# lmcinnes/pynndescent

Measured on AMD Instinct MI355X. Metric: index build: points indexed/sec (recall@10 vs brute force reported alongside), higher is better.
Workload: dtype f32

## Files before the change

include/pynnd_amd.h:

```cpp
#ifndef PYNND_AMD_H
#define PYNND_AMD_H

#include <stdint.h>

#ifdef __cplusplus
extern "C" {
#endif

#define NND_METRIC_SQEUCLIDEAN 0
#define NND_METRIC_ALT_COSINE 1
#define NND_METRIC_ALT_DOT 2
#define NND_METRIC_ALT_INNER_PRODUCT 3
#define NND_METRIC_CORRELATION 4
#define NND_METRIC_ALT_HELLINGER 5
enum { NND_METRIC_PROXY_INNER_PRODUCT = 6 };
enum {
    NND_METRIC_JACCARD = 8,
    NND_METRIC_DICE = 9,
    NND_METRIC_SOKALSNEATH = 10,
    NND_METRIC_MATCHING = 11,
    NND_METRIC_ROGERSTANIMOTO = 12,
    NND_METRIC_SOKALMICHENER = 13,
    NND_METRIC_KULSINSKI = 14,
    NND_METRIC_RUSSELLRAO = 15,
// ... 12 lines not shown
    int32_t n_trees;
    int32_t leaf_size;
    int32_t max_depth;
    int32_t max_candidates;
    int32_t n_iters;
    float delta;
    int64_t rng_state[3];
    int64_t tree_rng[3];
    int32_t device;
    int32_t join_blocks;
    int32_t flags;
    int32_t reserved[5];
} nnd_params;

#define NND_FLAG_NO_GRAPH 1
#define NND_FLAG_NO_PREP 2
#define NND_FLAG_TEST_SELECT_WAVE 4
#define NND_FLAG_TEST_SMALL_REGIONS 8
#define NND_FLAG_TEST_ROUTE_PLAIN 16
#define NND_FLAG_TEST_FOREST_BY_TREE 32
#define NND_FLAG_TEST_FAIL 64
#define NND_FLAG_TEST_VANISH 128
#define NND_FLAG_TEST_SAMPLE_ATOMIC 256
#define NND_FLAG_TEST_FOREST_FALLBACK_TOPS 512
#define NND_FLAG_TEST_FOREST_FALLBACK_SHARE 1024
#define NND_TEST_FALLBACK_AT(flags) ((((flags) & 512) ? 1 : 0) + (((flags) & 1024) ? 2 : 0))
#define NND_FLAG_TEST_SAMPLE_NOMEM 2048
#define NND_FLAG_TEST_SELECT_HALF 4096
#define NND_FLAG_TEST_GATHER_INLINE 8192
#define NND_FLAG_TEST_JOIN_UNSTAGED 16384

#define NND_FLAG_TEST_EXACT_F64 32768
#define NND_FLAG_TEST_RANDOM_INIT_ROWWISE 65536

typedef struct nnd_stats {
    int64_t n_iters_run;
    int64_t n_leaves;
    int64_t tree_levels;
    int64_t leaf_pairs;
    int64_t leaf_rows;
    int64_t join_pairs[64];
    int64_t join_rows[64];
    int64_t join_active[64];
    int64_t proposals[64];
    int64_t updates[64];
    float ms_prep, ms_forest, ms_leaf_init, ms_random_init, ms_descent, ms_finalize;
    float ms_sample[64], ms_join[64], ms_merge[64];
    int64_t join_mfma[64];
    int64_t leaf_mfma;
    int64_t n_cells;
    int64_t join_substeps[64];
} nnd_stats;

int32_t nnd_abi_version(void);
const char *nnd_last_global_error(void);
const char *nnd_last_error(nnd_handle_t h);

int32_t nnd_create(nnd_handle_t *out, const nnd_params *params);
int32_t nnd_destroy(nnd_handle_t h);
int32_t nnd_release_pending(void);

int32_t nnd_host_copy(void *dst, const void *src, int64_t bytes);
int32_t nnd_host_sqrt_f32(float *dst, const float *src, int64_t count);
void *nnd_host_alloc(int64_t bytes);
int32_t nnd_host_free(void *p);

// ... 254 lines not shown
```

pynndescent_amd/_capi.py:

```python
import ctypes as C
import os

import numpy as np

_HERE = os.path.dirname(os.path.abspath(__file__))
LIB_PATH = os.environ.get("PYNND_AMD_LIB", os.path.join(_HERE, "libpynnd_amd.so"))

NND_METRIC_SQEUCLIDEAN = 0
NND_METRIC_ALT_COSINE = 1
NND_METRIC_ALT_DOT = 2
NND_METRIC_ALT_INNER_PRODUCT = 3
NND_METRIC_CORRELATION = 4
NND_METRIC_ALT_HELLINGER = 5
NND_METRIC_PROXY_INNER_PRODUCT = 6
METRIC_CODES = {"euclidean": NND_METRIC_SQEUCLIDEAN, "l2": NND_METRIC_SQEUCLIDEAN, "sqeuclidean": NND_METRIC_SQEUCLIDEAN,
                "cosine": NND_METRIC_ALT_COSINE, "dot": NND_METRIC_ALT_DOT, "inner_product": NND_METRIC_ALT_INNER_PRODUCT,
                "correlation": NND_METRIC_CORRELATION, "hellinger": NND_METRIC_ALT_HELLINGER,
                "proxy_inner_product": NND_METRIC_PROXY_INNER_PRODUCT}
(NND_METRIC_JACCARD, NND_METRIC_DICE, NND_METRIC_SOKALSNEATH, NND_METRIC_MATCHING, NND_METRIC_ROGERSTANIMOTO,
 NND_METRIC_SOKALMICHENER, NND_METRIC_KULSINSKI, NND_METRIC_RUSSELLRAO, NND_METRIC_YULE) = range(8, 17)
BOOLEAN_METRIC_CODES = {"jaccard": NND_METRIC_JACCARD, "dice": NND_METRIC_DICE, "sokalsneath": NND_METRIC_SOKALSNEATH,
                        "matching": NND_METRIC_MATCHING, "rogerstanimoto": NND_METRIC_ROGERSTANIMOTO,
                        "sokalmichener": NND_METRIC_SOKALMICHENER, "kulsinski": NND_METRIC_KULSINSKI,
                        "russellrao": NND_METRIC_RUSSELLRAO, "yule": NND_METRIC_YULE}


def metric_code(name):
    return METRIC_CODES[name] if name in METRIC_CODES else BOOLEAN_METRIC_CODES[name]
NND_DTYPE_FLOAT32, NND_DTYPE_FLOAT16, NND_DTYPE_BFLOAT16, NND_DTYPE_FLOAT64 = 0, 1, 2, 3
NND_FILTER_MASK, NND_FILTER_IDS = 0, 1
NND_QUERY_FORMS = {"float": 0, "proxy": 1, "rerank": 2}
NND_CORRECT_COPY, NND_CORRECT_SQRT, NND_CORRECT_ALT_COSINE, NND_CORRECT_ALT_INNER_PRODUCT, NND_CORRECT_ALT_HELLINGER = 0, 1, 2, 3, 4
NND_LINEAR_DIAGONAL, NND_LINEAR_DENSE = 0, 1
NND_FLAG_NO_GRAPH = 1
NND_FLAG_NO_PREP = 2
NND_FLAG_TEST_SELECT_WAVE = 4
NND_FLAG_TEST_SMALL_REGIONS = 8
NND_FLAG_TEST_ROUTE_PLAIN = 16
NND_FLAG_TEST_FOREST_BY_TREE = 32
NND_FLAG_TEST_FAIL = 64
NND_FLAG_TEST_VANISH = 128
NND_FLAG_TEST_FOREST_FALLBACK_TOPS = 512
NND_FLAG_TEST_FOREST_FALLBACK_SHARE = 1024
NND_FLAG_TEST_GATHER_INLINE = 8192
NND_FLAG_TEST_JOIN_UNSTAGED = 16384
NND_FLAG_TEST_SELECT_HALF = 4096
NND_FLAG_TEST_SAMPLE_NOMEM = 2048
NND_FLAG_TEST_EXACT_F64 = 32768
NND_FLAG_TEST_RANDOM_INIT_ROWWISE = 65536
NND_FLAG_TEST_SAMPLE_ATOMIC = 256


class NNDParams(C.Structure):
    _fields_ = [
        ("n", C.c_int64),
        ("dim", C.c_int32),
        ("metric", C.c_int32),
        ("n_neighbors", C.c_int32),
        ("n_trees", C.c_int32),
        ("leaf_size", C.c_int32),
        ("max_depth", C.c_int32),
        ("max_candidates", C.c_int32),
        ("n_iters", C.c_int32),
        ("delta", C.c_float),
        ("rng_state", C.c_int64 * 3),
        ("tree_rng", C.c_int64 * 3),
        ("device", C.c_int32),
        ("join_blocks", C.c_int32),
        ("flags", C.c_int32),
        ("reserved", C.c_int32 * 5),
    ]


class NNDSearchGraphStats(C.Structure):
    _fields_ = [("forward_nnz", C.c_int64), ("reverse_nnz", C.c_int64), ("union_nnz", C.c_int64), ("final_nnz", C.c_int64),
                ("min_distance", C.c_float), ("max_degree_out", C.c_int32), ("ms_device", C.c_float), ("reserved", C.c_int32 * 3)]


class NNDStats(C.Structure):
    _fields_ = [
        ("n_iters_run", C.c_int64),
        ("n_leaves", C.c_int64),
# ... 972 lines not shown
```

pynndescent_amd/csrc/merge.h:

```cpp
#pragma once
#include "common.h"

#define NND_MAX_K 64

__device__ __forceinline__ uint64_t nnd_readlane_u64(uint64_t v, int src_lane) {
    uint32_t lo = (uint32_t)__builtin_amdgcn_readlane((int)(uint32_t)v, src_lane);
    uint32_t hi = (uint32_t)__builtin_amdgcn_readlane((int)(uint32_t)(v >> 32), src_lane);
    return ((uint64_t)hi << 32) | lo;
}

template <int NCHUNK, typename CandFn>
__device__ __forceinline__ int nnd_merge_row_regs(uint32_t *__restrict__ row_e, float *__restrict__ row_d,
                                                  float *__restrict__ th_slot, uint32_t e, float d, int k, int ncand,
                                                  CandFn cand) {
    const int lane = nnd_lane();
    const uint64_t mykey = (e == NND_EMPTY_E) ? NND_EMPTY_KEY : nnd_make_key(d, e);
    const uint32_t myidx = e & NND_IDX_MASK;
    const float th = __int_as_float(__builtin_amdgcn_readlane(__float_as_int(d), k - 1));
    const int nlist = __popcll(__ballot(e != NND_EMPTY_E));

    uint32_t cid[NCHUNK];
    float cd[NCHUNK];
    unsigned long long cmask[NCHUNK];
    int nv = 0;
// ... 178 lines not shown
            if (u) {
                pnext = __builtin_ctz(u);
                nlo = (uint32_t)__builtin_amdgcn_ds_bpermute((gbase + pnext) << 2, (int)clo);
                nhi = (uint32_t)__builtin_amdgcn_ds_bpermute((gbase + pnext) << 2, (int)chi);
            }
            const uint64_t mykey = ((uint64_t)khi << 32) | klo, ck = ((uint64_t)bhi << 32) | blo;
            const bool gt = mykey > ck;
            const int gtl = nnd_dpp_row_shr1(gt ? 1 : 0);
            const uint32_t llo = (uint32_t)nnd_dpp_row_shr1((int)klo), lhi = (uint32_t)nnd_dpp_row_shr1((int)khi);
            const uint32_t lfl = (uint32_t)nnd_dpp_row_shr1((int)flag);
            if (gt) {
                klo = gtl ? llo : blo;
                khi = gtl ? lhi : bhi;
                flag = gtl ? lfl : NND_NEW_BIT;
            }
        }
    }
    if (pushed == 0) return 0;
    const bool empty = (klo & khi) == 0xFFFFFFFFu;
    e = empty ? NND_EMPTY_E : (klo | flag);
    d = empty ? INFINITY : __uint_as_float(khi);
    return pushed;
}

template <int NBLK, typename CandFn>
__device__ __forceinline__ int nnd_merge_rows_q16(bool row_on, uint32_t *__restrict__ row_e, float *__restrict__ row_d,
                                                  float *__restrict__ th_slot, uint32_t e, float d, int k, int ncand,
                                                  CandFn cand) {
    const int j = nnd_lane() & 15;
    const uint32_t e_in = e;
    const float d_in = d;
    const int pushed = nnd_merge_rows_q16_regs<NBLK>(row_on, e, d, k, ncand, cand);
    if (pushed == 0) return 0;
    if (row_on && j < k && (e != e_in || d != d_in)) {
        row_e[j] = e;
        row_d[j] = d;
        if (j == k - 1) *th_slot = d;
    }
    return pushed;
}

#define NND_Q16B_CAP 32
#define NND_DPP_QUAD_XOR1 0xB1
#define NND_DPP_QUAD_XOR2 0x4E
#define NND_DPP_QUAD_MIRROR 0x1B
#define NND_DPP_ROW_MIRROR 0x140
#define NND_DPP_ROW_HALF_MIRROR 0x141
#define NND_DPP_ROW_SHL(n) (0x100 + (n))

template <int CTRL>
__device__ __forceinline__ uint32_t nnd_q16_partner(uint32_t v) {
    if constexpr (CTRL >= 0) {
        return (uint32_t)__builtin_amdgcn_update_dpp(0, (int)v, CTRL, 0xF, 0xF, true);
    } else {
        const int t = __builtin_amdgcn_update_dpp(0, (int)v, NND_DPP_QUAD_MIRROR, 0xF, 0xF, true);
        return (uint32_t)__builtin_amdgcn_update_dpp(0, t, NND_DPP_ROW_HALF_MIRROR, 0xF, 0xF, true);
    }
}
template <int CTRL>
__device__ __forceinline__ void nnd_q16_cx(uint32_t &lo, uint32_t &hi, bool keep_max) {
    const uint32_t plo = nnd_q16_partner<CTRL>(lo), phi = nnd_q16_partner<CTRL>(hi);
    const bool less = (((uint64_t)phi << 32) | plo) < (((uint64_t)hi << 32) | lo);
    const bool take = less != keep_max;
    lo = take ? plo : lo;
    hi = take ? phi : hi;
}
// ... 308 lines not shown
```

pynndescent_amd/csrc/merge.hip:

```cpp
#include "common.h"
#include "metric.h"
#include "merge.h"
#include "state.h"

__global__ __launch_bounds__(256) void k_merge(uint64_t *__restrict__ pbuf, uint8_t *__restrict__ pdirty, int pcap,
                                               int64_t lo, int64_t n, int k, int ks, uint32_t *__restrict__ knn_e,
                                               float *__restrict__ knn_d, float *__restrict__ th,
                                               long long *__restrict__ counters) {
    __shared__ int wacc[4];
    const int lane = nnd_lane(), w = threadIdx.x >> 6;
    const int64_t base = lo + ((int64_t)blockIdx.x * 4 + w) * 64;
    int acc = 0;
    unsigned long long m = 0;
    if (base < n) m = __ballot(base + lane < n && pdirty[base + lane < n ? base + lane : lo] != 0);
    struct pair_t {
        int64_t v[2];
        uint64_t key[2];
        uint32_t e[2];
        float d[2];
    };
    auto fetch = [&](pair_t &p) __attribute__((always_inline)) {
#pragma unroll
        for (int u = 0; u < 2; u++) {
            p.v[u] = -1;
// ... 13 lines not shown
    while (cur.v[0] >= 0) {
        if (m) fetch(nxt);
        else nxt.v[0] = nxt.v[1] = -1;
#pragma unroll
        for (int u = 0; u < 2; u++) {
            if (cur.v[u] < 0) continue;
            const int64_t v = cur.v[u];
            const uint64_t mykey = cur.key[u];
            acc += nnd_merge_row_regs<1>(knn_e + v * ks, knn_d + v * ks, th + v, cur.e[u], cur.d[u], k, pcap,
                                         [&](int c, uint32_t &id, float &dc) {
                                             id = nnd_key_idx(mykey);
                                             dc = nnd_key_dist(mykey);
                                             return mykey != NND_EMPTY_KEY;
                                         });
            if (lane < pcap && mykey != NND_EMPTY_KEY) pbuf[v * pcap + lane] = NND_EMPTY_KEY;
            if (lane == 0) pdirty[v] = 0;
        }
        cur = nxt;
    }
    if (lane == 0) wacc[w] = acc;
    __syncthreads();
    if (threadIdx.x == 0) {
        const long long a = (long long)wacc[0] + wacc[1] + wacc[2] + wacc[3];
        if (a) nnd_count(counters, CNT_ACCEPT, a);
    }
}

__global__ __launch_bounds__(256) void k_merge_q(uint64_t *__restrict__ pbuf, uint8_t *__restrict__ pdirty, int64_t lo,
                                                 int64_t n, int k, int ks, uint32_t *__restrict__ knn_e,
                                                 float *__restrict__ knn_d, float *__restrict__ th,
                                                 long long *__restrict__ counters) {
    constexpr int PCAP = 64, NB = PCAP / 16;
    __shared__ int wacc[4];
    const int lane = nnd_lane(), w = threadIdx.x >> 6, j = lane & 15, grp = lane >> 4;
    const int64_t base = lo + ((int64_t)blockIdx.x * 4 + w) * 64;
    int acc = 0;
    unsigned long long m = 0;
    if (base < n) m = __ballot(base + lane < n && pdirty[base + lane < n ? base + lane : lo] != 0);
    struct quad_t {
        int64_t v;
        uint64_t key[NB];
        uint32_t e;
        float d;
    };
    auto fetch = [&](quad_t &q) __attribute__((always_inline)) {
        int64_t vg = -1;
#pragma unroll
        for (int g = 0; g < 4; g++) {
            if (m) {
                const int64_t v = base + __builtin_ctzll(m);
                m &= m - 1;
                if (grp == g) vg = v;
            }
        }
        q.v = vg;
        const int64_t vv = vg >= 0 ? vg : lo;
#pragma unroll
        for (int b = 0; b < NB; b++) q.key[b] = pbuf[vv * PCAP + b * 16 + j];
        q.e = j < k ? knn_e[vv * ks + j] : NND_EMPTY_E;
        q.d = j < k ? knn_d[vv * ks + j] : INFINITY;
    };
    quad_t cur, nxt;
    cur.v = nxt.v = -1;
    bool have = m != 0;
    if (have) fetch(cur);
    while (have) {
        have = m != 0;
        if (have) fetch(nxt);
        const bool on = cur.v >= 0;
        const int64_t v = on ? cur.v : lo;
        const uint32_t e0 = on ? cur.e : NND_EMPTY_E;
        const float d0 = on ? cur.d : INFINITY;
        acc += nnd_merge_rows_q16<NB>(on, knn_e + v * ks, knn_d + v * ks, th + v, e0, d0, k, PCAP,
                                      [&](int c, uint32_t &id, float &dc) {
                                          const int b = c >> 4;
                                          const uint64_t kk = b == 0 ? cur.key[0] : (b == 1 ? cur.key[1] : (b == 2 ? cur.key[2] : cur.key[3]));
                                          id = nnd_key_idx(kk);
                                          dc = nnd_key_dist(kk);
                                          return kk != NND_EMPTY_KEY;
                                      });
        if (on) {
#pragma unroll
            for (int b = 0; b < NB; b++)
                if (cur.key[b] != NND_EMPTY_KEY) pbuf[v * PCAP + b * 16 + j] = NND_EMPTY_KEY;
            if (j == 0) pdirty[v] = 0;
        }
        cur = nxt;
    }
    if (lane == 0) wacc[w] = acc;
    __syncthreads();
    if (threadIdx.x == 0) {
        const long long a = (long long)wacc[0] + wacc[1] + wacc[2] + wacc[3];
        if (a) nnd_count(counters, CNT_ACCEPT, a);
    }
}

__global__ __launch_bounds__(256) void k_merge_wide(uint64_t *__restrict__ pbuf, uint8_t *__restrict__ pdirty, int pcap, int64_t lo, int64_t n,
                                                    int k, int ks, uint32_t *__restrict__ knn_e, float *__restrict__ knn_d,
                                                    float *__restrict__ th, long long *__restrict__ counters) {
    __shared__ uint64_t scr[4][NND_WIDE_SCRATCH_WORDS];
    __shared__ int wacc[4];
    const int lane = nnd_lane(), w = threadIdx.x >> 6;
    const int64_t base = lo + ((int64_t)blockIdx.x * 4 + w) * 64;
    int acc = 0;
    unsigned long long m = 0;
    if (base < n) m = __ballot(base + lane < n && pdirty[base + lane < n ? base + lane : lo] != 0);
    while (m) {
        const int64_t v = base + __builtin_ctzll(m);
        m &= m - 1;
        const uint64_t mykey = lane < pcap ? pbuf[v * pcap + lane] : NND_EMPTY_KEY;
        acc += nnd_merge_row_lds<1>(scr[w], knn_e + v * ks, knn_d + v * ks, th + v, k, pcap, [&](int c, uint32_t &id, float &dc) {
            id = nnd_key_idx(mykey);
            dc = nnd_key_dist(mykey);
// ... 482 lines not shown
```

pynndescent_amd/csrc/sample.hip:

```cpp
#include "common.h"
#include "state.h"

__device__ __forceinline__ uint32_t nnd_offer_salt(uint32_t it_seed, uint32_t u) { return nnd_hash2(it_seed ^ 0x3C6EF372u, u); }

__device__ __forceinline__ uint32_t nnd_offer_slot(uint32_t salt_u, uint32_t v, int rcap) { return nnd_hash2(salt_u ^ 0x68E31DA4u, v) & (uint32_t)(rcap - 1); }
__device__ __forceinline__ int64_t nnd_offer_addr(uint32_t u, uint32_t cls, uint32_t salt_u, uint32_t v, int rcap, int wide) {
    return wide ? (int64_t)u * 2 * rcap + nnd_offer_slot(salt_u, v, 2 * rcap) : ((int64_t)u * 2 + cls) * rcap + nnd_offer_slot(salt_u, v, rcap);
}
__device__ __forceinline__ uint64_t nnd_offer_key(uint32_t slot_word, uint32_t salt_u) {
    return ((uint64_t)slot_word << 32) | (uint64_t)(nnd_unmix32(slot_word) ^ salt_u);
}

__global__ __launch_bounds__(256) void k_sample_reverse(const uint32_t *__restrict__ knn_e, int64_t row_lo, int64_t n, int k, int ks, uint32_t it_seed,
                                                        uint32_t *__restrict__ rbuf, int rcap, int64_t own_lo, int64_t own_hi, int pass,
                                                        uint8_t *__restrict__ active, const int32_t *__restrict__ order, int wide) {
    int64_t b = blockIdx.x;
    if ((gridDim.x & 7) == 0) b = (b & 7) * (gridDim.x >> 3) + (b >> 3);
    const int64_t g = row_lo + b * blockDim.y + threadIdx.y;
    const int j = threadIdx.x;
    if (g >= n || j >= k) return;
    const int64_t v = order ? (int64_t)order[g] : g;
    uint32_t e = knn_e[v * ks + j];
    if (e == NND_EMPTY_E) return;
    uint32_t u = e & NND_IDX_MASK;
// ... 512 lines not shown
    uint32_t *slots = rbuf + vv * 2 * RCAP;
    if (act) {
        rw0 = slots[j];
        rw1 = slots[RCAP + j];
        if (rw0 != NND_EMPTY_SLOT) slots[j] = NND_EMPTY_SLOT;
        if (rw1 != NND_EMPTY_SLOT) slots[RCAP + j] = NND_EMPTY_SLOT;
    }
    nnd_select_half<WIDE>(knn_e, k, ks, mc, mcp, it_seed, cand, vv, act, e, rw0, rw1, sk, j, hb);
}

#define RV_TAB 1024
#ifndef RV_RPT
#define RV_RPT 8
#endif
#define RV_NOHASH 0xFFFFu
#ifndef RV_SEL_THREADS
#define RV_SEL_THREADS 512
#endif

__device__ __forceinline__ uint32_t rv_tab_hash(uint32_t b) { return (b * 2654435761u) >> 22; }

__device__ __forceinline__ int rv_tab_find(volatile uint32_t *hkey, uint32_t b) {
    uint32_t h = rv_tab_hash(b);
#pragma unroll 1
    for (int p = 0; p < 24; p++) {
        uint32_t cur = hkey[h];
        if (cur == 0xFFFFFFFFu) cur = atomicCAS((uint32_t *)&hkey[h], 0xFFFFFFFFu, b);
        if (cur == 0xFFFFFFFFu || cur == b) return (int)h;
        h = (h + 1) & (RV_TAB - 1);
    }
    return -1;
}
#define RV_NOKEY 0xFFFFFFFFu
__device__ __forceinline__ void rv_row_groups(uint32_t key, int &rank, int &size, int &leader) {
    const int lane = (int)__builtin_amdgcn_mbcnt_hi(~0u, __builtin_amdgcn_mbcnt_lo(~0u, 0u));
    rank = 0;
    size = 1;
    leader = lane;
#define RV_ROT(r)                                                                         \
    {                                                                                     \
        const uint32_t ok = (uint32_t)nnd_dpp_i32<NND_DPP_ROW_ROR(r)>((int)key);           \
        const int ol = nnd_dpp_i32<NND_DPP_ROW_ROR(r)>(lane);                              \
        const bool eq = ok == key;                                                        \
        size += eq ? 1 : 0;                                                               \
        rank += (eq && ol < lane) ? 1 : 0;                                                \
        leader = (eq && ol < leader) ? ol : leader;                                       \
    }
    RV_ROT(1) RV_ROT(2) RV_ROT(3) RV_ROT(4) RV_ROT(5) RV_ROT(6) RV_ROT(7) RV_ROT(8)
    RV_ROT(9) RV_ROT(10) RV_ROT(11) RV_ROT(12) RV_ROT(13) RV_ROT(14) RV_ROT(15)
#undef RV_ROT
}
__device__ __forceinline__ uint32_t rv_offer_word(uint32_t it_seed, uint32_t u, uint32_t v) { return nnd_mix32(v ^ nnd_offer_salt(it_seed, u)); }

__global__ __launch_bounds__(256) void k_rev_mark(const uint32_t *__restrict__ knn_e, int64_t row0, int64_t n_rows, int ks, uint8_t *__restrict__ active) {
    const int64_t i = ((int64_t)blockIdx.x * 256 + threadIdx.x) * 4;
    if (i >= n_rows * ks) return;
    const u32x4 e = *(const u32x4 *)(knn_e + row0 * ks + i);
    const int64_t v = row0 + i / ks;
#pragma unroll
    for (int q = 0; q < 4; q++) {
        const uint32_t w = e[q];
        if (w != NND_EMPTY_E && (w >> 31)) {
            active[v] = 1;
            const uint32_t t = w & NND_IDX_MASK;
            if ((uint32_t)(t - (uint32_t)row0) < (uint32_t)n_rows) active[t] = 1;
        }
    }
}
__global__ void k_rev_mark_records(const int32_t *__restrict__ targets, int64_t count, int64_t row0, int64_t n_rows, uint8_t *__restrict__ active) {
    const int64_t i = (int64_t)blockIdx.x * blockDim.x + threadIdx.x;
    if (i >= count) return;
    const uint32_t t = (uint32_t)targets[i];
    const uint32_t u = t & NND_IDX_MASK;
    if ((t >> 31) && (uint32_t)(u - (uint32_t)row0) < (uint32_t)n_rows) active[u] = 1;
}

struct rv_inbox {
    const uint32_t *cursor = nullptr;
    const uint2 *rec = nullptr;
    int cap = 0;
    const uint2 *ov = nullptr;
    const uint32_t *ov_count = nullptr;
};
__global__ __launch_bounds__(256) void k_rev_place(const uint32_t *__restrict__ knn_e, int64_t row0, int64_t n, int k, int ks, uint32_t it_seed,
                                                   const int32_t *__restrict__ order, const int32_t *__restrict__ pos, int logB,
                                                   uint8_t *__restrict__ active, int mark, uint32_t *__restrict__ in_cursor,
                                                   uint2 *__restrict__ in_rec, int cap, uint2 *__restrict__ ov, uint32_t *__restrict__ ov_count) {
    __shared__ uint32_t hkey[RV_TAB], hcnt[RV_TAB], hbase[RV_TAB];
    const int tid = threadIdx.y * blockDim.x + threadIdx.x;
    for (int i = tid; i < RV_TAB; i += 256) { hkey[i] = 0xFFFFFFFFu; hcnt[i] = 0; }
    __syncthreads();
    const int j = threadIdx.x;
    const uint32_t sub = blockIdx.x & 7u, bmask = (1u << logB) - 1u;
    uint32_t ev[RV_RPT], vv[RV_RPT];
#pragma unroll
    for (int it = 0; it < RV_RPT; it++) {
        const int64_t g = ((int64_t)blockIdx.x * RV_RPT + it) * blockDim.y + threadIdx.y;
        ev[it] = NND_EMPTY_E;
        vv[it] = 0;
        if (g < n && j < k) {
            vv[it] = (uint32_t)(order ? order[g] : (int32_t)(row0 + g));
            ev[it] = knn_e[(int64_t)vv[it] * ks + j];
        }
    }
    uint32_t bb[RV_RPT], w[RV_RPT], at[RV_RPT];
    uint16_t m[RV_RPT], hh[RV_RPT];
#pragma unroll
    for (int it = 0; it < RV_RPT; it++) {
        bb[it] = RV_NOKEY;
        w[it] = at[it] = 0;
        m[it] = 0;
        hh[it] = RV_NOHASH;
        if (ev[it] != NND_EMPTY_E && (uint32_t)((ev[it] & NND_IDX_MASK) - (uint32_t)row0) >= (uint32_t)n) {
            if ((ev[it] >> 31) && mark == 1) active[vv[it]] = 1;
            ev[it] = NND_EMPTY_E;
        }
        if (ev[it] != NND_EMPTY_E) {
            const uint32_t u = ev[it] & NND_IDX_MASK, cls = ev[it] >> 31;
            if (cls && mark == 1) { active[vv[it]] = 1; active[u] = 1; }
            if (mark == 2 && !cls && !active[u]) ev[it] = NND_EMPTY_E;
        }
        if (ev[it] != NND_EMPTY_E) {
            const uint32_t u = ev[it] & NND_IDX_MASK, cls = ev[it] >> 31;
            const uint32_t ul = u - (uint32_t)row0;
            const uint32_t p = (uint32_t)(pos ? pos[ul] : (int32_t)ul);
            bb[it] = p >> logB;
            w[it] = rv_offer_word(it_seed, u, vv[it]);
            m[it] = (uint16_t)((p & bmask) | (cls << 15));
        }
    }
#pragma unroll
    for (int it = 0; it < RV_RPT; it++) {
        int rank, size, leader;
        rv_row_groups(bb[it], rank, size, leader);
        int h = -1;
        uint32_t base = 0;
        if (bb[it] != RV_NOKEY && rank == 0) {
            h = rv_tab_find(hkey, bb[it]);
            base = h >= 0 ? atomicAdd(&hcnt[h], (uint32_t)size) : atomicAdd(&in_cursor[(size_t)bb[it] * 8 + sub], (uint32_t)size);
        }
        h = __shfl(h, leader, 64);
        base = (uint32_t)__shfl((int)base, leader, 64);
        if (bb[it] != RV_NOKEY) {
            hh[it] = h >= 0 ? (uint16_t)h : RV_NOHASH;
            at[it] = base + (uint32_t)rank;
        }
    }
    __syncthreads();
    for (int i = tid; i < RV_TAB; i += 256)
        if (hcnt[i]) hbase[i] = atomicAdd(&in_cursor[(size_t)hkey[i] * 8 + sub], hcnt[i]);
    __syncthreads();
#pragma unroll
    for (int it = 0; it < RV_RPT; it++) {
        if (bb[it] == RV_NOKEY) continue;
        const uint32_t at_ = hh[it] == RV_NOHASH ? at[it] : hbase[hh[it]] + at[it];
        if (at_ < (uint32_t)cap)
            in_rec[((size_t)bb[it] * 8 + sub) * cap + at_] = make_uint2(w[it], (uint32_t)m[it]);
        else
            ov[atomicAdd(ov_count, 1u)] = make_uint2(w[it], (bb[it] << 9) | (((uint32_t)m[it] >> 15) << 8) | ((uint32_t)m[it] & 0xFFu));
    }
}
__global__ __launch_bounds__(256) void k_rev_import(const int32_t *__restrict__ targets, const uint32_t *__restrict__ sources, int64_t count,
                                                    uint32_t it_seed, int64_t row0, int64_t n, const int32_t *__restrict__ pos, int logB,
                                                    const uint8_t *__restrict__ active, int filter, uint32_t *__restrict__ in_cursor,
                                                    uint2 *__restrict__ in_rec, int cap, uint2 *__restrict__ ov, uint32_t *__restrict__ ov_count) {
    const int64_t i = (int64_t)blockIdx.x * 256 + threadIdx.x;
    if (i >= count) return;
    const uint32_t t = (uint32_t)targets[i];
    const uint32_t cls = t >> 31, u = t & NND_IDX_MASK, ul = u - (uint32_t)row0;
    if (ul >= (uint32_t)n || (filter && !cls && !active[u])) return;
    const uint32_t p = (uint32_t)(pos ? pos[ul] : (int32_t)ul);
    const uint32_t b = p >> logB, tl = p & ((1u << logB) - 1u);
    const uint32_t w = rv_offer_word(it_seed, u, sources[i]);
    const size_t sr = (size_t)b * 8 + (threadIdx.x & 7);
    const uint32_t at = atomicAdd(&in_cursor[sr], 1u);
    if (at < (uint32_t)cap) {
        in_rec[sr * cap + at] = make_uint2(w, tl | (cls << 15));
    } else {
        ov[atomicAdd(ov_count, 1u)] = make_uint2(w, (b << 9) | (cls << 8) | tl);
    }
}
template <typename F>
__device__ __forceinline__ void rv_each_record(const rv_inbox &ib, int64_t b, int tid, int nthr, F f) {
    uint32_t c[8], pre[9];
    bool over = false;
#pragma unroll
    for (int sr = 0; sr < 8; sr++) c[sr] = ib.cursor[b * 8 + sr];
    pre[0] = 0;
#pragma unroll
    for (int sr = 0; sr < 8; sr++) {
        over = over || c[sr] > (uint32_t)ib.cap;
        pre[sr + 1] = pre[sr] + (c[sr] < (uint32_t)ib.cap ? c[sr] : (uint32_t)ib.cap);
    }
    const uint2 *base = ib.rec + (size_t)b * 8 * ib.cap;
    for (uint32_t i = tid; i < pre[8]; i += nthr) {
        int sr = 0;
#pragma unroll
        for (int q = 1; q < 8; q++) sr += i >= pre[q] ? 1 : 0;
        uint32_t lo = pre[0];
#pragma unroll
        for (int q = 1; q < 8; q++) lo = sr >= q ? pre[q] : lo;
        const uint2 r = base[(size_t)sr * ib.cap + (i - lo)];
        f(r.x, r.y);
    }
    if (over) {
        const uint32_t M = *ib.ov_count;
        for (uint32_t i = tid; i < M; i += nthr) {
            const uint2 r = ib.ov[i];
            if ((int64_t)(r.y >> 9) == b) f(r.x, (r.y & 0xFFu) | (((r.y >> 8) & 1u) << 15));
        }
    }
}

__device__ __forceinline__ uint32_t rv_ovf_slot(uint32_t word, uint32_t cap) { return nnd_mix32(word ^ 0x68E31DA4u) & (cap - 1u); }

template <int RCAP, int NB, bool WIDE>
__global__ __launch_bounds__(1024) void k_rev_fill(rv_inbox ib, int64_t row0, int64_t n, const int32_t *__restrict__ order,
                                                   const uint8_t *__restrict__ active, uint32_t *__restrict__ rbuf) {
    constexpr int ROW = 2 * RCAP;
    constexpr int CAP = WIDE ? 2 * RCAP : RCAP;
    constexpr int NBANK = WIDE ? NB : 2 * NB;
    __shared__ uint32_t bank[NB * ROW];
    __shared__ uint32_t cnt[NBANK];
    __shared__ int any_ovf;
    const int tid = threadIdx.x;
    const int64_t b = blockIdx.x;
    for (int i = tid; i < NB * ROW; i += 1024) bank[i] = NND_EMPTY_SLOT;
    for (int i = tid; i < NBANK; i += 1024) cnt[i] = 0;
    if (tid == 0) any_ovf = 0;
    __syncthreads();
    rv_each_record(ib, b, tid, 1024, [&](uint32_t w, uint32_t m) {
        const uint32_t bk = WIDE ? (m & 0x7FFFu) : ((m & 0x7FFFu) * 2 + (m >> 15));
        const uint32_t s = atomicAdd(&cnt[bk], 1u);
        if (s < (uint32_t)CAP) bank[bk * CAP + s] = w;
    });
    __syncthreads();
// ... 56 lines not shown
            if (lane == 0) {
                acnt[tid >> 6] = __popcll(am);
                icnt[tid >> 6] = __popcll(im);
            }
        }
    }
    for (int i = tid; i < NB * ROW; i += NT) bank[i] = NND_EMPTY_SLOT;
    for (int i = tid; i < NBANK; i += NT) cnt[i] = 0;
    if (tid == 0) any_ovf = 0;
    __syncthreads();
    int nact = NB, rounds = PER;
    uint32_t tpk = 0;
    if constexpr (LW == 16) {
        static_assert(PER <= 4 && NB <= 256, "a byte per target, a word per group");
        const int c0 = acnt[0];
        nact = c0 + acnt[1];
        rounds = (nact + NG - 1) / NG;
#pragma unroll
        for (int r = 0; r < PER; r++) {
            const int idx = r * NG + grp;
            if (idx < nact) tpk |= (uint32_t)(idx < c0 ? alist[0][idx] : alist[1][idx - c0]) << (8 * r);
        }
    }
    auto has_target = [&](int r) -> bool { return LW == 32 || r * NG + grp < nact; };
    auto target_of = [&](int r) -> int {
        if constexpr (LW == 16) return (int)((tpk >> (8 * r)) & 0xFFu);
        return r * NG + grp;
    };
    uint32_t pre_e = NND_EMPTY_E;
    if (rounds > 0) {
        const int32_t v0 = has_target(0) ? vtx[target_of(0)] : -1;
        if (v0 >= 0 && j < k) pre_e = knn_e[(int64_t)v0 * ks + j];
    }
    rv_each_record(ib, b, tid, NT, [&](uint32_t w, uint32_t m) {
        const uint32_t bk = WIDE ? (m & 0x7FFFu) : ((m & 0x7FFFu) * 2 + (m >> 15));
        const uint32_t sl = atomicAdd(&cnt[bk], 1u);
        if (sl < (uint32_t)CAP) bank[bk * CAP + sl] = w;
    });
    __syncthreads();
    for (int i = tid; i < NBANK; i += NT)
        if (cnt[i] > (uint32_t)CAP) any_ovf = 1;
    __syncthreads();
    if (any_ovf) {
        for (int i = tid; i < NBANK * CAP; i += NT)
            if (cnt[i / CAP] > (uint32_t)CAP) bank[i] = NND_EMPTY_SLOT;
        __syncthreads();
        rv_each_record(ib, b, tid, NT, [&](uint32_t w, uint32_t m) {
            const uint32_t bk = WIDE ? (m & 0x7FFFu) : ((m & 0x7FFFu) * 2 + (m >> 15));
            if (cnt[bk] > (uint32_t)CAP) atomicMin(&bank[bk * CAP + rv_ovf_slot(w, CAP)], w);
        });
        __syncthreads();
    }
    uint64_t *sk = skey[grp];
    if constexpr (LW == 16) {
        const int todo = icnt[0] + icnt[1] ? NB * LW : 0;
        for (int i = tid; i < todo; i += NT) {
            const int32_t v = vtx[i / LW];
            if (v <= -2)
                for (int q = i % LW; q < mcp; q += LW) cand[(int64_t)(-2 - v) * 2 * mcp + q] = -1;
        }
    }
#pragma unroll 1
    for (int r = 0; r < rounds; r++) {
        const int tl = target_of(r);
        const int32_t v = has_target(r) ? vtx[tl] : -1;
        const bool act = v >= 0;
        const uint32_t e = pre_e;
// ... 107 lines not shown
    return 0;
}

static bool rv_fused(const nnd_ctx *ctx) {
    return ctx->k <= 32 && ctx->rcap == 32 && ctx->mc <= 32 && !(ctx->p.flags & NND_FLAG_TEST_SELECT_WAVE);
}
static bool rv_bucketed(const nnd_ctx *ctx) { return (ctx->rcap == 32 || ctx->rcap == 64) && !ctx->rv_off && !(ctx->p.flags & NND_FLAG_TEST_SAMPLE_ATOMIC); }
static int launch_sample_bucketed(nnd_ctx *ctx, uint32_t it_seed, bool wide, const int32_t *in_targets, const uint32_t *in_sources, int64_t n_in) {
    const bool fused = rv_fused(ctx), shard = ctx->n_ranks > 1;
    const int logB = (fused || ctx->rcap != 32) ? 7 : 8;
    const int64_t row0 = shard ? ctx->own_lo : 0, n_rows = shard ? ctx->own_hi - ctx->own_lo : ctx->n;
    if (n_rows <= 0) return 0;
    const int32_t *order = shard ? ctx->own_order : ((ctx->forest_built && ctx->p.n_trees > 0) ? ctx->perm[ctx->cur] : nullptr);
    int cap = 0;
    if (const int prc = rv_prepare(ctx, logB, order, row0, n_rows, n_in, &cap)) return prc;
    const int32_t *pos = order ? ctx->rv_pos : nullptr;
    const int64_t nb = ((n_rows - 1) >> logB) + 1;
    if (nb >= ((int64_t)1 << 23)) { ctx->set_error("candidate sampling: %lld buckets exceed the 2^23 bucket ids of an overflow record", (long long)nb); return 1; }
    int ksp = 16;
    while (ksp < ctx->ks) ksp <<= 1;
    const int rows = 256 / ksp;
    const unsigned grid = (unsigned)((n_rows + (int64_t)rows * RV_RPT - 1) / ((int64_t)rows * RV_RPT));
    hipStream_t st = ctx->stream;
    uint32_t *ov_count = ctx->rv_in_cursor + (size_t)nb * 8;
    NND_HIP_CHECK(hipMemsetAsync(ctx->rv_in_cursor, 0, sizeof(uint32_t) * ((size_t)nb * 8 + 8), st));
    NND_HIP_CHECK(hipMemsetAsync(ctx->active + row0, ctx->all_new ? 1 : 0, (size_t)n_rows, st));
    int mark = ctx->all_new ? 0 : 1;
    if (mark == 1 && (shard || (ctx->last_updates >= 0 && ctx->last_updates * 8 < ctx->n * ctx->k))) {
        hipLaunchKernelGGL(k_rev_mark, dim3((unsigned)((n_rows * ctx->ks / 4 + 255) / 256)), dim3(256), 0, st, ctx->knn_e, row0, n_rows, ctx->ks, ctx->active);
        if (n_in > 0)
            hipLaunchKernelGGL(k_rev_mark_records, dim3((unsigned)((n_in + 255) / 256)), dim3(256), 0, st, in_targets, n_in, row0, n_rows, ctx->active);
        mark = 2;
    }
    hipLaunchKernelGGL(k_rev_place, dim3(grid), dim3(ksp, rows), 0, st, ctx->knn_e, row0, n_rows, ctx->k, ctx->ks, it_seed, order, pos, logB, ctx->active,
                       mark, ctx->rv_in_cursor, ctx->rv_in_rec, cap, ctx->rv_ov, ov_count);
    if (n_in > 0)
        hipLaunchKernelGGL(k_rev_import, dim3((unsigned)((n_in + 255) / 256)), dim3(256), 0, st, in_targets, in_sources, n_in, it_seed, row0, n_rows, pos, logB,
                           ctx->active, mark == 2 ? 1 : 0, ctx->rv_in_cursor, ctx->rv_in_rec, cap, ctx->rv_ov, ov_count);
    rv_inbox ib;
    ib.cursor = ctx->rv_in_cursor;
    ib.rec = ctx->rv_in_rec;
    ib.cap = cap;
    ib.ov = ctx->rv_ov;
    ib.ov_count = ov_count;
    if (fused) {
        const bool q16 = ctx->ks == 16 && ctx->mc <= 16 && ctx->mcp == 16 && !(ctx->p.flags & NND_FLAG_TEST_SELECT_HALF);
        auto kern = q16 ? (wide ? k_rev_select<true, 16> : k_rev_select<false, 16>) : (wide ? k_rev_select<true, 32> : k_rev_select<false, 32>);
        hipLaunchKernelGGL(kern, dim3((unsigned)nb), dim3(RV_SEL_THREADS), 0, st, ib, row0, n_rows, order, ctx->active, ctx->knn_e, ctx->k, ctx->ks, ctx->mc, ctx->mcp,
                           it_seed, ctx->cand);
        return 0;
    }
    ctx->rbuf_clean = false;
    auto fill = ctx->rcap == 32 ? (wide ? k_rev_fill<32, 256, true> : k_rev_fill<32, 256, false>) : k_rev_fill<64, 128, false>;
    hipLaunchKernelGGL(fill, dim3((unsigned)nb), dim3(1024), 0, st, ib, row0, n_rows, order, ctx->active, ctx->rbuf);
    launch_select(ctx, it_seed, wide);
    return 0;
}

int nnd_launch_sample(nnd_ctx *ctx) {
    if (ctx->n_ranks > 1) {
        ctx->set_error("nnd_launch_sample: this handle is one shard of a row-sharded build; use nnd_sample_begin / nnd_sample_finish");
        return 1;
    }
    const uint32_t it_seed = sample_seed(ctx);
    if (rv_bucketed(ctx)) {
        const bool wide_b = sample_wide(ctx);
        const int brc = launch_sample_bucketed(ctx, it_seed, wide_b, nullptr, nullptr, 0);
// ... 148 lines not shown
```

Baseline: 55.10 million.

## Restructure reverse-neighbour placement loads, batch inbox reads, and compact merge candidates via LDS

The merge kernel now compacts the candidate keys that pass the threshold into a per-wave LDS queue, then merges them in blocks of 16 using a ds_bpermute broadcast with a duplicate check, so candidates that cannot enter the list are dropped first. The reverse-placement kernel now issues its order, knn and pos loads in separate unconditional batches, and computes row-group rank, size and leader from one DPP-built bitmask instead of per-step tracking. The select kernel reads inbox records in batches of four per thread to keep several loads in flight. A plain atomic placement kernel is added behind a test flag as a reference path. These changes add LDS use and register pressure, and the clamped loads may touch memory the old code skipped.

```diff
diff --git a/include/pynnd_amd.h b/include/pynnd_amd.h
--- a/include/pynnd_amd.h
+++ b/include/pynnd_amd.h
@@ -68,6 +68,7 @@
 
 #define NND_FLAG_TEST_EXACT_F64 32768
 #define NND_FLAG_TEST_RANDOM_INIT_ROWWISE 65536
+#define NND_FLAG_TEST_PLACE_PLAIN 131072
 
 typedef struct nnd_stats {
     int64_t n_iters_run;
diff --git a/pynndescent_amd/_capi.py b/pynndescent_amd/_capi.py
--- a/pynndescent_amd/_capi.py
+++ b/pynndescent_amd/_capi.py
@@ -48,6 +48,7 @@
 NND_FLAG_TEST_SAMPLE_NOMEM = 2048
 NND_FLAG_TEST_EXACT_F64 = 32768
 NND_FLAG_TEST_RANDOM_INIT_ROWWISE = 65536
+NND_FLAG_TEST_PLACE_PLAIN = 131072
 NND_FLAG_TEST_SAMPLE_ATOMIC = 256
 
 
diff --git a/pynndescent_amd/csrc/merge.h b/pynndescent_amd/csrc/merge.h
--- a/pynndescent_amd/csrc/merge.h
+++ b/pynndescent_amd/csrc/merge.h
@@ -234,6 +234,96 @@
     const float d_in = d;
     const int pushed = nnd_merge_rows_q16_regs<NBLK>(row_on, e, d, k, ncand, cand);
     if (pushed == 0) return 0;
+    if (row_on && j < k && (e != e_in || d != d_in)) {
+        row_e[j] = e;
+        row_d[j] = d;
+        if (j == k - 1) *th_slot = d;
+    }
+    return pushed;
+}
+
+template <int NB>
+__device__ __forceinline__ int nnd_merge_rows_q16_slots(bool row_on, uint32_t *__restrict__ row_e, float *__restrict__ row_d,
+                                                        float *__restrict__ th_slot, uint32_t e, float d, int k,
+                                                        const uint64_t (&slot)[NB], uint64_t *wave_q) {
+    const int lane = nnd_lane(), j = lane & 15, gbase = lane & 48;
+    const uint32_t e_in = e;
+    const float d_in = d;
+    uint32_t klo = e & NND_IDX_MASK, khi = __float_as_uint(d);
+    if (e == NND_EMPTY_E) { klo = 0xFFFFFFFFu; khi = 0xFFFFFFFFu; }
+    uint32_t flag = e == NND_EMPTY_E ? 0u : (e & NND_NEW_BIT);
+    const uint32_t myidx = e & NND_IDX_MASK;
+    const float th = __int_as_float(__builtin_amdgcn_ds_bpermute((gbase + k - 1) << 2, __float_as_int(d)));
+    const bool any_list = __ballot(e != NND_EMPTY_E) != 0;
+    const uint32_t below = (1u << j) - 1u;
+    uint64_t *my = wave_q + (lane >> 4) * (16 * NB);
+    bool ok[NB];
+    int at[NB], ns = 0;
+    unsigned long long any = 0;
+#pragma unroll
+    for (int b = 0; b < NB; b++) {
+        ok[b] = row_on && slot[b] != NND_EMPTY_KEY && nnd_key_dist(slot[b]) < th;
+        const unsigned long long bm = __ballot(ok[b]);
+        const uint32_t m16 = (uint32_t)(bm >> gbase) & 0xFFFFu;
+        at[b] = ns + __popc(m16 & below);
+        ns += __popc(m16);
+        any |= bm;
+    }
+    if (!any) return 0;
+#pragma unroll
+    for (int b = 0; b < NB; b++)
+        if (ok[b]) my[at[b]] = slot[b];
+    nnd_wave_lds_sync();
+    int pushed = 0;
+#pragma unroll 1
+    for (int blk = 0; blk < NB; blk++) {
+        if (!__ballot(ns > 16 * blk)) break;
+        const uint64_t ck = my[16 * blk + j];
+        const uint32_t cid = (uint32_t)ck;
+        bool okc = 16 * blk + j < ns;
+        if (any_list) {
+            uint32_t rid = myidx;
+            bool dup = false;
+#pragma unroll
+            for (int t = 0; t < 16; t++) {
+                dup |= rid == cid;
+                rid = (uint32_t)nnd_dpp_row_ror1((int)rid);
+            }
+            okc = okc && !dup;
+        }
+        const unsigned long long mask = __ballot(okc);
+        if (!mask) continue;
+        pushed += __popcll(mask);
+        const uint32_t clo = okc ? cid : 0xFFFFFFFFu, chi = okc ? (uint32_t)(ck >> 32) : 0xFFFFFFFFu;
+        uint32_t u = (uint32_t)(mask | (mask >> 16) | (mask >> 32) | (mask >> 48)) & 0xFFFFu;
+        int pnext = __builtin_ctz(u);
+        uint32_t nlo = (uint32_t)__builtin_amdgcn_ds_bpermute((gbase + pnext) << 2, (int)clo);
+        uint32_t nhi = (uint32_t)__builtin_amdgcn_ds_bpermute((gbase + pnext) << 2, (int)chi);
+        while (u) {
+            const uint32_t blo = nlo, bhi = nhi;
+            u &= u - 1;
+            if (u) {
+                pnext = __builtin_ctz(u);
+                nlo = (uint32_t)__builtin_amdgcn_ds_bpermute((gbase + pnext) << 2, (int)clo);
+                nhi = (uint32_t)__builtin_amdgcn_ds_bpermute((gbase + pnext) << 2, (int)chi);
+            }
+            const uint64_t mykey = ((uint64_t)khi << 32) | klo, bk = ((uint64_t)bhi << 32) | blo;
+            const bool gt = mykey > bk;
+            const int gtl = nnd_dpp_row_shr1(gt ? 1 : 0);
+            const uint32_t llo = (uint32_t)nnd_dpp_row_shr1((int)klo), lhi = (uint32_t)nnd_dpp_row_shr1((int)khi);
+            const uint32_t lfl = (uint32_t)nnd_dpp_row_shr1((int)flag);
+            if (gt) {
+                klo = gtl ? llo : blo;
+                khi = gtl ? lhi : bhi;
+                flag = gtl ? lfl : NND_NEW_BIT;
+            }
+        }
+    }
+    nnd_wave_lds_sync();
+    if (pushed == 0) return 0;
+    const bool empty = (klo & khi) == 0xFFFFFFFFu;
+    e = empty ? NND_EMPTY_E : (klo | flag);
+    d = empty ? INFINITY : __uint_as_float(khi);
     if (row_on && j < k && (e != e_in || d != d_in)) {
         row_e[j] = e;
         row_d[j] = d;
diff --git a/pynndescent_amd/csrc/merge.hip b/pynndescent_amd/csrc/merge.hip
--- a/pynndescent_amd/csrc/merge.hip
+++ b/pynndescent_amd/csrc/merge.hip
@@ -69,6 +69,7 @@
                                                  long long *__restrict__ counters) {
     constexpr int PCAP = 64, NB = PCAP / 16;
     __shared__ int wacc[4];
+    __shared__ uint64_t queue[4][4 * PCAP];
     const int lane = nnd_lane(), w = threadIdx.x >> 6, j = lane & 15, grp = lane >> 4;
     const int64_t base = lo + ((int64_t)blockIdx.x * 4 + w) * 64;
     int acc = 0;
@@ -108,14 +109,7 @@
         const int64_t v = on ? cur.v : lo;
         const uint32_t e0 = on ? cur.e : NND_EMPTY_E;
         const float d0 = on ? cur.d : INFINITY;
-        acc += nnd_merge_rows_q16<NB>(on, knn_e + v * ks, knn_d + v * ks, th + v, e0, d0, k, PCAP,
-                                      [&](int c, uint32_t &id, float &dc) {
-                                          const int b = c >> 4;
-                                          const uint64_t kk = b == 0 ? cur.key[0] : (b == 1 ? cur.key[1] : (b == 2 ? cur.key[2] : cur.key[3]));
-                                          id = nnd_key_idx(kk);
-                                          dc = nnd_key_dist(kk);
-                                          return kk != NND_EMPTY_KEY;
-                                      });
+        acc += nnd_merge_rows_q16_slots<NB>(on, knn_e + v * ks, knn_d + v * ks, th + v, e0, d0, k, cur.key, queue[w]);
         if (on) {
 #pragma unroll
             for (int b = 0; b < NB; b++)
diff --git a/pynndescent_amd/csrc/sample.hip b/pynndescent_amd/csrc/sample.hip
--- a/pynndescent_amd/csrc/sample.hip
+++ b/pynndescent_amd/csrc/sample.hip
@@ -568,23 +568,17 @@
     return -1;
 }
 #define RV_NOKEY 0xFFFFFFFFu
-__device__ __forceinline__ void rv_row_groups(uint32_t key, int &rank, int &size, int &leader) {
-    const int lane = (int)__builtin_amdgcn_mbcnt_hi(~0u, __builtin_amdgcn_mbcnt_lo(~0u, 0u));
-    rank = 0;
-    size = 1;
-    leader = lane;
-#define RV_ROT(r)                                                                         \
-    {                                                                                     \
-        const uint32_t ok = (uint32_t)nnd_dpp_i32<NND_DPP_ROW_ROR(r)>((int)key);           \
-        const int ol = nnd_dpp_i32<NND_DPP_ROW_ROR(r)>(lane);                              \
-        const bool eq = ok == key;                                                        \
-        size += eq ? 1 : 0;                                                               \
-        rank += (eq && ol < lane) ? 1 : 0;                                                \
-        leader = (eq && ol < leader) ? ol : leader;                                       \
-    }
+__device__ __forceinline__ void rv_row_groups(uint32_t key, int lane, int &rank, int &size, int &leader) {
+    const uint32_t j = (uint32_t)lane & 15u, walk = 0x10001u << j;
+    uint32_t mask = walk;
+#define RV_ROT(r) mask |= ((uint32_t)nnd_dpp_i32<NND_DPP_ROW_ROR(r)>((int)key) == key) ? (walk >> (r)) : 0u;
     RV_ROT(1) RV_ROT(2) RV_ROT(3) RV_ROT(4) RV_ROT(5) RV_ROT(6) RV_ROT(7) RV_ROT(8)
     RV_ROT(9) RV_ROT(10) RV_ROT(11) RV_ROT(12) RV_ROT(13) RV_ROT(14) RV_ROT(15)
 #undef RV_ROT
+    mask &= 0xFFFFu;
+    size = __popc(mask);
+    rank = __popc(mask & ((1u << j) - 1u));
+    leader = (lane & ~15) + (__ffs((int)mask) - 1);
 }
 __device__ __forceinline__ uint32_t rv_offer_word(uint32_t it_seed, uint32_t u, uint32_t v) { return nnd_mix32(v ^ nnd_offer_salt(it_seed, u)); }
 
@@ -629,46 +623,70 @@
     const int j = threadIdx.x;
     const uint32_t sub = blockIdx.x & 7u, bmask = (1u << logB) - 1u;
     uint32_t ev[RV_RPT], vv[RV_RPT];
+    const int jk = j < k ? j : 0;
 #pragma unroll
     for (int it = 0; it < RV_RPT; it++) {
         const int64_t g = ((int64_t)blockIdx.x * RV_RPT + it) * blockDim.y + threadIdx.y;
-        ev[it] = NND_EMPTY_E;
-        vv[it] = 0;
-        if (g < n && j < k) {
-            vv[it] = (uint32_t)(order ? order[g] : (int32_t)(row0 + g));
-            ev[it] = knn_e[(int64_t)vv[it] * ks + j];
-        }
-    }
+        vv[it] = (uint32_t)(g < n ? g : n - 1);
+    }
+    if (order) {
+#pragma unroll
+        for (int it = 0; it < RV_RPT; it++) vv[it] = (uint32_t)order[vv[it]];
+    } else {
+#pragma unroll
+        for (int it = 0; it < RV_RPT; it++) vv[it] += (uint32_t)row0;
+    }
+#pragma unroll
+    for (int it = 0; it < RV_RPT; it++) ev[it] = knn_e[(int64_t)vv[it] * ks + jk];
     uint32_t bb[RV_RPT], w[RV_RPT], at[RV_RPT];
     uint16_t m[RV_RPT], hh[RV_RPT];
+#pragma unroll
+    for (int it = 0; it < RV_RPT; it++) {
+        const int64_t g = ((int64_t)blockIdx.x * RV_RPT + it) * blockDim.y + threadIdx.y;
+        if (!(g < n && j < k)) ev[it] = NND_EMPTY_E;
+        if (ev[it] != NND_EMPTY_E && (uint32_t)((ev[it] & NND_IDX_MASK) - (uint32_t)row0) >= (uint32_t)n) {
+            if ((ev[it] >> 31) && mark == 1) active[vv[it]] = 1;
+            ev[it] = NND_EMPTY_E;
+        }
+    }
+    if (mark == 1) {
+#pragma unroll
+        for (int it = 0; it < RV_RPT; it++)
+            if (ev[it] != NND_EMPTY_E && (ev[it] >> 31)) {
+                active[vv[it]] = 1;
+                active[ev[it] & NND_IDX_MASK] = 1;
+            }
+    } else if (mark == 2) {
+        uint8_t au[RV_RPT];
+#pragma unroll
+        for (int it = 0; it < RV_RPT; it++) au[it] = active[ev[it] != NND_EMPTY_E ? (ev[it] & NND_IDX_MASK) : vv[it]];
+#pragma unroll
+        for (int it = 0; it < RV_RPT; it++)
+            if (ev[it] != NND_EMPTY_E && !(ev[it] >> 31) && !au[it]) ev[it] = NND_EMPTY_E;
+    }
+    uint32_t pp[RV_RPT];
+#pragma unroll
+    for (int it = 0; it < RV_RPT; it++) {
+        const uint32_t ul = ev[it] != NND_EMPTY_E ? (ev[it] & NND_IDX_MASK) - (uint32_t)row0 : 0u;
+        pp[it] = (uint32_t)(pos ? pos[ul] : (int32_t)ul);
+    }
 #pragma unroll
     for (int it = 0; it < RV_RPT; it++) {
         bb[it] = RV_NOKEY;
         w[it] = at[it] = 0;
         m[it] = 0;
         hh[it] = RV_NOHASH;
-        if (ev[it] != NND_EMPTY_E && (uint32_t)((ev[it] & NND_IDX_MASK) - (uint32_t)row0) >= (uint32_t)n) {
-            if ((ev[it] >> 31) && mark == 1) active[vv[it]] = 1;
-            ev[it] = NND_EMPTY_E;
-        }
         if (ev[it] != NND_EMPTY_E) {
             const uint32_t u = ev[it] & NND_IDX_MASK, cls = ev[it] >> 31;
-            if (cls && mark == 1) { active[vv[it]] = 1; active[u] = 1; }
-            if (mark == 2 && !cls && !active[u]) ev[it] = NND_EMPTY_E;
-        }
-        if (ev[it] != NND_EMPTY_E) {
-            const uint32_t u = ev[it] & NND_IDX_MASK, cls = ev[it] >> 31;
-            const uint32_t ul = u - (uint32_t)row0;
-            const uint32_t p = (uint32_t)(pos ? pos[ul] : (int32_t)ul);
-            bb[it] = p >> logB;
+            bb[it] = pp[it] >> logB;
             w[it] = rv_offer_word(it_seed, u, vv[it]);
-            m[it] = (uint16_t)((p & bmask) | (cls << 15));
+            m[it] = (uint16_t)((pp[it] & bmask) | (cls << 15));
         }
     }
 #pragma unroll
     for (int it = 0; it < RV_RPT; it++) {
         int rank, size, leader;
-        rv_row_groups(bb[it], rank, size, leader);
+        rv_row_groups(bb[it], tid & 63, rank, size, leader);
         int h = -1;
         uint32_t base = 0;
         if (bb[it] != RV_NOKEY && rank == 0) {
@@ -694,6 +712,36 @@
             in_rec[((size_t)bb[it] * 8 + sub) * cap + at_] = make_uint2(w[it], (uint32_t)m[it]);
         else
             ov[atomicAdd(ov_count, 1u)] = make_uint2(w[it], (bb[it] << 9) | (((uint32_t)m[it] >> 15) << 8) | ((uint32_t)m[it] & 0xFFu));
+    }
+}
+__global__ __launch_bounds__(256) void k_rev_plain(const uint32_t *__restrict__ knn_e, int64_t row0, int64_t n, int k, int ks, uint32_t it_seed,
+                                                   const int32_t *__restrict__ order, const int32_t *__restrict__ pos, int logB,
+                                                   uint8_t *__restrict__ active, int mark, uint32_t *__restrict__ in_cursor,
+                                                   uint2 *__restrict__ in_rec, int cap, uint2 *__restrict__ ov, uint32_t *__restrict__ ov_count) {
+    const int j = threadIdx.x;
+    if (j >= k) return;
+    for (int it = 0; it < RV_RPT; it++) {
+        const int64_t g = ((int64_t)blockIdx.x * RV_RPT + it) * blockDim.y + threadIdx.y;
+        if (g >= n) continue;
+        const uint32_t v = (uint32_t)(order ? order[g] : (int32_t)(row0 + g));
+        const uint32_t e = knn_e[(int64_t)v * ks + j];
+        if (e == NND_EMPTY_E) continue;
+        const uint32_t u = e & NND_IDX_MASK, cls = e >> 31, ul = u - (uint32_t)row0;
+        if (ul >= (uint32_t)n) {
+            if (cls && mark == 1) active[v] = 1;
+            continue;
+        }
+        if (cls && mark == 1) { active[v] = 1; active[u] = 1; }
+        if (mark == 2 && !cls && !active[u]) continue;
+        const uint32_t p = (uint32_t)(pos ? pos[ul] : (int32_t)ul);
+        const uint32_t b = p >> logB, tl = p & ((1u << logB) - 1u);
+        const uint32_t w = rv_offer_word(it_seed, u, v);
+        const size_t sr = (size_t)b * 8 + (blockIdx.x & 7u);
+        const uint32_t at = atomicAdd(&in_cursor[sr], 1u);
+        if (at < (uint32_t)cap)
+            in_rec[sr * cap + at] = make_uint2(w, tl | (cls << 15));
+        else
+            ov[atomicAdd(ov_count, 1u)] = make_uint2(w, (b << 9) | (cls << 8) | (tl & 0xFFu));
     }
 }
 __global__ __launch_bounds__(256) void k_rev_import(const int32_t *__restrict__ targets, const uint32_t *__restrict__ sources, int64_t count,
@@ -738,6 +786,50 @@
         for (int q = 1; q < 8; q++) lo = sr >= q ? pre[q] : lo;
         const uint2 r = base[(size_t)sr * ib.cap + (i - lo)];
         f(r.x, r.y);
+    }
+    if (over) {
+        const uint32_t M = *ib.ov_count;
+        for (uint32_t i = tid; i < M; i += nthr) {
+            const uint2 r = ib.ov[i];
+            if ((int64_t)(r.y >> 9) == b) f(r.x, (r.y & 0xFFu) | (((r.y >> 8) & 1u) << 15));
+        }
+    }
+}
+
+#define RV_BATCH 4
+template <typename F>
+__device__ __forceinline__ void rv_each_record_batched(const rv_inbox &ib, int64_t b, int tid, int nthr, F f) {
+    uint32_t c[8], pre[9];
+    bool over = false;
+#pragma unroll
+    for (int sr = 0; sr < 8; sr++) c[sr] = ib.cursor[b * 8 + sr];
+    pre[0] = 0;
+#pragma unroll
+    for (int sr = 0; sr < 8; sr++) {
+        over = over || c[sr] > (uint32_t)ib.cap;
+        pre[sr + 1] = pre[sr] + (c[sr] < (uint32_t)ib.cap ? c[sr] : (uint32_t)ib.cap);
+    }
+    const uint2 *base = ib.rec + (size_t)b * 8 * ib.cap;
+    const uint32_t total = pre[8];
+    for (uint32_t i0 = 0; i0 < total; i0 += RV_BATCH * nthr) {
+        uint2 r[RV_BATCH];
+#pragma unroll
+        for (int q = 0; q < RV_BATCH; q++) {
+            r[q] = make_uint2(0u, 0u);
+            if (i0 + q * nthr >= total) continue;
+            uint32_t i = i0 + q * nthr + tid;
+            i = i < total ? i : total - 1u;
+            int sr = 0;
+#pragma unroll
+            for (int s = 1; s < 8; s++) sr += i >= pre[s] ? 1 : 0;
+            uint32_t lo = pre[0];
+#pragma unroll
+            for (int s = 1; s < 8; s++) lo = sr >= s ? pre[s] : lo;
+            r[q] = base[(size_t)sr * ib.cap + (i - lo)];
+        }
+#pragma unroll
+        for (int q = 0; q < RV_BATCH; q++)
+            if (i0 + q * nthr + tid < total) f(r[q].x, r[q].y);
     }
     if (over) {
         const uint32_t M = *ib.ov_count;
@@ -860,7 +952,7 @@
         const int32_t v0 = has_target(0) ? vtx[target_of(0)] : -1;
         if (v0 >= 0 && j < k) pre_e = knn_e[(int64_t)v0 * ks + j];
     }
-    rv_each_record(ib, b, tid, NT, [&](uint32_t w, uint32_t m) {
+    rv_each_record_batched(ib, b, tid, NT, [&](uint32_t w, uint32_t m) {
         const uint32_t bk = WIDE ? (m & 0x7FFFu) : ((m & 0x7FFFu) * 2 + (m >> 15));
         const uint32_t sl = atomicAdd(&cnt[bk], 1u);
         if (sl < (uint32_t)CAP) bank[bk * CAP + sl] = w;
@@ -1034,7 +1126,7 @@
             hipLaunchKernelGGL(k_rev_mark_records, dim3((unsigned)((n_in + 255) / 256)), dim3(256), 0, st, in_targets, n_in, row0, n_rows, ctx->active);
         mark = 2;
     }
-    hipLaunchKernelGGL(k_rev_place, dim3(grid), dim3(ksp, rows), 0, st, ctx->knn_e, row0, n_rows, ctx->k, ctx->ks, it_seed, order, pos, logB, ctx->active,
+    hipLaunchKernelGGL((ctx->p.flags & NND_FLAG_TEST_PLACE_PLAIN) ? k_rev_plain : k_rev_place, dim3(grid), dim3(ksp, rows), 0, st, ctx->knn_e, row0, n_rows, ctx->k, ctx->ks, it_seed, order, pos, logB, ctx->active,
                        mark, ctx->rv_in_cursor, ctx->rv_in_rec, cap, ctx->rv_ov, ov_count);
     if (n_in > 0)
         hipLaunchKernelGGL(k_rev_import, dim3((unsigned)((n_in + 255) / 256)), dim3(256), 0, st, in_targets, in_sources, n_in, it_seed, row0, n_rows, pos, logB,
```

Result: no change. 54.88 million (-0.4%).
